# jackie840129/FedFR

Measured on AMD Instinct MI355X. Metric: images/sec (iresnet100+CosFace train step, bs=128/GPU, 112x112), higher is better.
Workload: dtype fp16; 1 GPU; iresnet100 + CosFace(s=30,m=0.4) + dense 1000-class cosine head, full train step (fwd+bwd+momentum-SGD), batch 128/GPU, 112x112 synthetic faces, random-init weights, fp16 activations/weights with fp32 accumulate + fp32 master weights, fp32 head; global_batch=128, parallelism=1 client per GPU (FedAvg), dp1, clients=1

## Files before the change

fedfr_amd/csrc/gemm_nt_glds.hip:

```cpp
#include "nt_epilogue.h"

#ifndef NT_GLDS_NS
#define NT_GLDS_NS 4
#endif
namespace {
template <int N_>
__device__ __forceinline__ void wait_vmcnt() {
  asm volatile("s_waitcnt vmcnt(%0)" ::"n"(N_) : "memory");
}

template <int BM, int BN, int WM, int WN, int NS, bool CONV>
__global__ __launch_bounds__(64 * WM * WN) void gemm_nt_glds_kernel(GemmNT p_) {
  GemmNT p = p_;
  if (p.par_on == 2) {
    const int cls = 3 - (int)blockIdx.z;
    p.par_h = cls >> 1; p.par_w = cls & 1;
    p.ksteps_total = (1 + p.par_h) * (1 + p.par_w) * p.cpt;
    p.ksteps_per_split = p.ksteps_total;
  }
  constexpr int NW = WM * WN, NT = 64 * NW;
  constexpr int TM = BM / WM / 16, TN = BN / WN / 16;
  constexpr int A_BYTES = BM * 128, B_BYTES = BN * 128, STAGE = A_BYTES + B_BYTES;
  constexpr int AP = (BM / 8) / NW, BP = (BN / 8) / NW, PER = AP + BP;
  constexpr int NRD = TM + TN, NM = TM * TN;
  static_assert((BM / 8) % NW == 0 && (BN / 8) % NW == 0 && NS >= 3 && NS <= 5 && AP >= 1 && BP >= 1, "tile geometry");
  typedef __attribute__((address_space(3))) void* lds_ptr_t;
  extern __shared__ __attribute__((aligned(1024))) unsigned char smem[];

  const int tid = threadIdx.x, lane = tid & 63;
  const int wave = __builtin_amdgcn_readfirstlane(tid >> 6);
  const int wm = wave / WN, wn = wave % WN;
  const int lid = xcd_remap(blockIdx.x, gridDim.x);
  const int bn = lid % p.nbn, bm = lid / p.nbn;
  const int split = blockIdx.y;
  const int m0 = bm * BM, n0 = bn * BN;
  const int kt0 = split * p.ksteps_per_split;
  const int kt1 = min(kt0 + p.ksteps_per_split, p.ksteps_total);

  const int prow = lane >> 3, pch = (lane & 7) ^ prow;
  constexpr unsigned OOB = 0xfffffff0u;
  int a_hb[AP], a_wb[AP];
  unsigned a_base[AP];
  bool a_ok[AP];
#pragma unroll
  for (int j = 0; j < AP; ++j) {
    const int m = m0 + (j * NW + wave) * 8 + prow;
    a_ok[j] = m < p.M;
    if (CONV) {
      const int mm = a_ok[j] ? m : 0;
      const int hw = p.Ho * p.Wo;
      const int img = mm / hw, rem = mm - img * hw;
      int ho = rem / p.Wo, wo = rem - ho * p.Wo;
      if (p.par_on) {
        ho = 2 * ho + p.par_h;
        wo = 2 * wo + p.par_w;
      }
      a_hb[j] = ho * p.stride - p.pad;
      a_wb[j] = wo * p.stride - p.pad;
      a_base[j] = ((unsigned)(img * p.H * p.W) * (unsigned)p.C + (unsigned)(pch * 8)) * 2u;
    } else {
      a_hb[j] = a_wb[j] = 0;
      a_base[j] = ((unsigned)(a_ok[j] ? m : 0) * (unsigned)p.lda + (unsigned)(pch * 8)) * 2u;
    }
  }
  unsigned b_base[BP];
  bool b_ok[BP];
#pragma unroll
  for (int j = 0; j < BP; ++j) {
    const int n = n0 + (j * NW + wave) * 8 + prow;
    b_ok[j] = n < p.N;
    b_base[j] = ((unsigned)(b_ok[j] ? n : 0) * (unsigned)p.K + (unsigned)(pch * 8)) * 2u;
  }
  int kti = kt0;
  int tap = kt0 / p.cpt, cc = kt0 - tap * p.cpt;
  int r = tap / p.S, s = tap - r * p.S;
  const int s0 = p.par_on ? 1 - p.par_w : 0, tstep = p.par_on ? 2 : 1;
  if (p.par_on) {
    const int nS = 1 + p.par_w;
    r = (1 - p.par_h) + 2 * (tap / nS);
    s = s0 + 2 * (tap % nS);
  }
  const __amdgpu_buffer_rsrc_t rsA = make_rsrc(p.A, p.a_bytes), rsB = make_rsrc(p.B, p.b_bytes);
  const int upm = p.up - 1, ups = p.up >> 1;
  const unsigned rowB = (unsigned)(p.W * p.C * 2), pixB = (unsigned)(p.C * 2);
  auto issue = [&](int slot) {
    unsigned char* sA = smem + slot * STAGE;
    unsigned char* sB = sA + A_BYTES;
    const bool live = kti < kt1;
    const unsigned kA = (unsigned)(CONV ? cc * 128 : kti * 128);
    const bool klive = live & (CONV | (kti * 64 + pch * 8 < p.K));
#pragma unroll
    for (int j = 0; j < AP; ++j) {
      bool ok = klive & a_ok[j];
      unsigned off = a_base[j] + kA;
      if (CONV) {
        int hp = a_hb[j] + r, wp = a_wb[j] + s;
        ok = ok & (((hp | wp) & upm) == 0);
        hp >>= ups;
        wp >>= ups;
        ok = ok & ((unsigned)hp < (unsigned)p.H) & ((unsigned)wp < (unsigned)p.W);
        off += __umul24((unsigned)hp, rowB) + __umul24((unsigned)wp, pixB);
      }
      __builtin_amdgcn_raw_ptr_buffer_load_lds(rsA, (lds_ptr_t)(sA + (j * NW + wave) * 1024), 16, (int)(ok ? off : OOB), 0, 0, 0);
    }
    const unsigned kB = (unsigned)(CONV ? ((r * p.S + s) * p.cpt + cc) * 128 : kti * 128);
#pragma unroll
    for (int j = 0; j < BP; ++j)
      __builtin_amdgcn_raw_ptr_buffer_load_lds(rsB, (lds_ptr_t)(sB + (j * NW + wave) * 1024), 16, (int)((klive & b_ok[j]) ? b_base[j] + kB : OOB), 0, 0, 0);
    ++kti;
    cc += 1;
    const bool wc = cc == p.cpt;
    cc = wc ? 0 : cc;
    s += wc ? tstep : 0;
    const bool ws = s >= p.S;
    s = ws ? s0 : s;
    r += ws ? tstep : 0;
  };

  const int l15 = lane & 15, lg = lane >> 4;
  int a_addr[TM], b_addr[TN];
#pragma unroll
  for (int mi = 0; mi < TM; ++mi) {
    const int row = wm * (BM / WM) + mi * 16 + l15;
    a_addr[mi] = row * 128 + ((lg ^ (row & 7)) << 4);
  }
#pragma unroll
  for (int ni = 0; ni < TN; ++ni) {
    const int row = wn * (BN / WN) + ni * 16 + l15;
    b_addr[ni] = A_BYTES + row * 128 + ((lg ^ (row & 7)) << 4);
  }
  f32x4_t acc[TN][TM];
#pragma unroll
  for (int a = 0; a < TN; ++a)
#pragma unroll
    for (int b = 0; b < TM; ++b) acc[a][b] = (f32x4_t){0.f, 0.f, 0.f, 0.f};
  bf16x8_t f0a[TM], f0b[TN], f1a[TM], f1b[TN];
  auto read_frags = [&](bf16x8_t (&fa)[TM], bf16x8_t (&fb)[TN], const unsigned char* st, int ks) {
#pragma unroll
    for (int ni = 0; ni < TN; ++ni) fb[ni] = *reinterpret_cast<const bf16x8_t*>(st + (b_addr[ni] ^ (ks * 64)));
#pragma unroll
    for (int mi = 0; mi < TM; ++mi) fa[mi] = *reinterpret_cast<const bf16x8_t*>(st + (a_addr[mi] ^ (ks * 64)));
  };
  auto mfma_all = [&](const bf16x8_t (&fa)[TM], const bf16x8_t (&fb)[TN]) {
#pragma unroll
    for (int ni = 0; ni < TN; ++ni)
#pragma unroll
      for (int mi = 0; mi < TM; ++mi) acc[ni][mi] = MFMA16(fb[ni], fa[mi], acc[ni][mi]);
  };

#pragma unroll
  for (int i = 0; i < NS - 1; ++i) issue(i);
  wait_vmcnt<(NS - 2) * PER>();
  __builtin_amdgcn_s_barrier();
  read_frags(f0a, f0b, smem, 0);
  int slot = 0;
  for (int kt = kt0; kt < kt1; ++kt) {
    const unsigned char* cur = smem + slot * STAGE;
    const int nslot = slot + 1 == NS ? 0 : slot + 1, fslot = slot == 0 ? NS - 1 : slot - 1;
    read_frags(f1a, f1b, cur, 1);
    mfma_all(f0a, f0b);
#pragma unroll
    for (int i = 0; i < NRD; ++i) {
      __builtin_amdgcn_sched_group_barrier(0x008, (NM / NRD) > 0 ? (NM / NRD) : 1, 0);
      __builtin_amdgcn_sched_group_barrier(0x100, 1, 0);
    }
    __builtin_amdgcn_sched_barrier(0);
    wait_vmcnt<(NS - 3) * PER>();
    __builtin_amdgcn_s_barrier();
    __builtin_amdgcn_sched_barrier(0);
    read_frags(f0a, f0b, smem + nslot * STAGE, 0);
    issue(fslot);
    mfma_all(f1a, f1b);
    constexpr int NE = NRD > PER ? NRD : PER, MP2 = (NM / NE) > 0 ? (NM / NE) : 1;
#pragma unroll
    for (int i = 0; i < NE; ++i) {
      __builtin_amdgcn_sched_group_barrier(0x008, MP2, 0);
      if (i < NRD) __builtin_amdgcn_sched_group_barrier(0x100, 1, 0);
      if (i < PER) __builtin_amdgcn_sched_group_barrier(0x020, 1, 0);
    }
    __builtin_amdgcn_sched_barrier(0);
    slot = nslot;
  }
  wait_vmcnt<0>();
  __syncthreads();
  nt_epilogue<BM, BN, WM, WN, NT>(p, acc, smem, bm, m0, n0, split, wm, wn, tid, lane);
}

template <int BM, int BN, int WM, int WN, int NS, bool CONV>
int launch_impl2(GemmNT p, int splits, int slot, hipStream_t st) {
  const int nbm = ceil_div(p.M, BM);
  p.nbn = ceil_div(p.N, BN);
  p.ksteps_per_split = ceil_div(p.ksteps_total, splits);
  FEDFR_REQUIRE(ceil_div(p.ksteps_total, p.ksteps_per_split) == splits, "gemm_nt_glds: splits=%d leaves an empty split (ksteps=%d)", splits,
                p.ksteps_total);
  constexpr size_t kRing = (size_t)NS * (BM + BN) * 128, kEpi = (size_t)BM * (BN * 2 + 16);
  constexpr size_t lds = kRing > kEpi ? kRing : kEpi;
  static PerDeviceOnce attr_once;
  attr_once.run([&] {
    hipFuncSetAttribute(reinterpret_cast<const void*>(&gemm_nt_glds_kernel<BM, BN, WM, WN, NS, CONV>), hipFuncAttributeMaxDynamicSharedMemorySize, (int)lds);
  });
  const dim3 grid(nbm * p.nbn, splits, p.par_on == 2 ? 4 : 1);
  ProfScope prof(slot, 2.0 * p.M * p.N * (p.par_on == 2 ? 64.0 * 9 * p.cpt : p.par_on ? 64.0 * p.ksteps_total : (double)p.K), st, gemm_nt_alg_bytes(p, splits));
  hipLaunchKernelGGL((gemm_nt_glds_kernel<BM, BN, WM, WN, NS, CONV>), grid, dim3(64 * WM * WN), lds, st, p);
  FEDFR_LAUNCH_CHECK("gemm_nt_glds");
  return FEDFR_OK;
}
template <int BM, int BN, int WM, int WN, int NS>
int launch_impl(const GemmNT& p, int splits, int slot, hipStream_t st) {
  if (p.mode == 1) {
    FEDFR_REQUIRE((long long)p.W * p.C * 2 < (1 << 24) && p.H < (1 << 15), "gemm_nt_glds: image row too large for the 24-bit address multiplies");
    return launch_impl2<BM, BN, WM, WN, NS, true>(p, splits, slot, st);
  }
  return launch_impl2<BM, BN, WM, WN, NS, false>(p, splits, slot, st);
}
}

int g_nt_glds = 4;

bool gemm_nt_glds_applies(const GemmNT& p, int BM, int splits) {
  const bool pays = (g_nt_glds & 8) || (!p.par_on && ceil_div(p.ksteps_total, splits) >= 16);
  return (g_nt_glds & 7) > 0 && p.N > 64 && (BM == 128 || BM == 64) && pays && !p.bpart && !p.esc && !p.eadd && !p.Cb2;
}

int launch_nt_glds(const GemmNT& p, int BM, int splits, int slot, hipStream_t st) {
  FEDFR_REQUIRE(gemm_nt_glds_applies(p, BM, splits), "gemm_nt_glds: unsupported problem");
  const int v = g_nt_glds & 7;
  const bool up = v >= 3 && BM == 64 && (!p.stats || ceil_div(p.M, 64) == 2 * ceil_div(p.M, 128));
  if (BM == 128 || up) return (v & 1) == 0 ? launch_impl<128, 128, 2, 4, NT_GLDS_NS>(p, splits, slot, st) : launch_impl<128, 128, 2, 2, 4>(p, splits, slot, st);
  return launch_impl<64, 128, 1, 4, 3>(p, splits, slot, st);
}
```

fedfr_amd/csrc/wgrad9.hip:

```cpp
#include "gemm_tn_dev.h"
#ifndef W9_READS_FIRST
#define W9_READS_FIRST 0
#endif
#ifndef W9_ABLATE
#define W9_ABLATE 0
#endif

int g_wgrad9 = 1;

namespace {
template <int N_>
__device__ __forceinline__ void w9_wait_vmcnt() {
  asm volatile("s_waitcnt vmcnt(%0)" ::"n"(N_) : "memory");
}
__device__ __forceinline__ int w9_swz(int row) { return (((row >> 1) & 1) << 1) | (((row >> 3) & 1) << 2); }

struct W9 {
  const bf16_t* dy;
  const bf16_t* x;
  float* out;
  int cout, cin, nci;
  int ntiles;
  int nstages, per_split;
  int W, lg;
  unsigned dy_bytes, x_bytes;
};

template <int W_, int R_, int LOG_PW>
__global__ __launch_bounds__(512) __attribute__((amdgpu_waves_per_eu(3, 3))) void wgrad9_kernel(W9 p) {
  constexpr int PW = 1 << LOG_PW, KP = R_ * PW, KS = KP / 32;
  constexpr int VG = PW / 16, WIN = 2 + 2 * VG, NG = 2 * KS + 2 * VG;
  constexpr int BANDS = W_ / R_;
  constexpr int P_PIECES = KP / 16;
  constexpr int Q_ROWS = (NG * 16 + 2 + 7) / 8 * 8, Q_PIECES = Q_ROWS / 8;
  constexpr int NP = P_PIECES + Q_PIECES, NPW = (NP + 7) / 8;
  constexpr int P_B = KP * 64, Q_B = Q_ROWS * 128, STAGE_B = P_B + Q_B;
  static_assert(KP % 32 == 0 && W_ % R_ == 0 && W_ <= PW && (R_ + 2) * PW + 2 <= Q_ROWS, "band geometry");
  static_assert(P_B % 1024 == 0 && (NG - 1) * 2048 < 65536, "ds_read immediate offsets");
  typedef __attribute__((address_space(3))) void* lds_ptr_t;
  typedef __attribute__((address_space(3))) unsigned char* lds_uc_t;
  extern __shared__ __attribute__((aligned(1024))) unsigned char smem[];

  const int tid = threadIdx.x, lane = tid & 63;
  const int wave = __builtin_amdgcn_readfirstlane(tid >> 6);
  const int cb = wave >> 1, ch = wave & 1;
  const int lid = xcd_remap((int)blockIdx.x, (int)gridDim.x);
  const int split = lid / p.ntiles, tile = lid - split * p.ntiles;
  const int tco = tile / p.nci, tci = tile - tco * p.nci;
  const int co0 = tco * 32, ci0 = tci * 64;
  const int s0 = split * p.per_split;
  const int nst = min(p.per_split, p.nstages - s0);

  const __amdgpu_buffer_rsrc_t rsP = make_rsrc(p.dy, p.dy_bytes), rsQ = make_rsrc(p.x, p.x_bytes);
  constexpr unsigned OOB = 0xfffffff0u;
  const int prow = lane >> 3;
  auto issue_stage = [&](int s, int buf) {
    const int per_img = BANDS << (2 * p.lg);
    const int img = s / per_img, rem = s - img * per_img;
    const int sub = rem / BANDS, band = rem - sub * BANDS;
    const int y0 = (sub >> p.lg) * W_ + band * R_, x0 = (sub & ((1 << p.lg) - 1)) * W_;
    const int Wi = p.W;
#pragma unroll
    for (int j = 0; j < NPW; ++j) {
      const int piece = min(j * 8 + wave, NP - 1);
      if (piece < P_PIECES) {
        const int r = piece * 16 + (lane >> 2);
        const int yl = r >> LOG_PW, xx = r & (PW - 1);
        const bool ok = s >= 0 && xx < W_;
        const unsigned off = ((unsigned)((img * Wi + y0 + yl) * Wi + x0 + xx) * (unsigned)p.cout + (unsigned)(co0 + (lane & 3) * 8)) * 2u;
        __builtin_amdgcn_raw_ptr_buffer_load_lds(rsP, (lds_ptr_t)(smem + buf * STAGE_B + piece * 1024), 16, (int)(ok ? off : OOB), 0, 0, 0);
      } else {
        const int qp = piece - P_PIECES;
        const int r = qp * 8 + prow;
        const int ql = r >> LOG_PW, xx = r & (PW - 1);
        const int lc = (lane & 7) ^ w9_swz(r);
        const int y = y0 + ql - 1, xc = x0 + xx - 1;
        const bool ok = s >= 0 && ql < R_ + 2 && xx < W_ + 2 && (unsigned)y < (unsigned)Wi && (unsigned)xc < (unsigned)Wi;
        const unsigned off = ((unsigned)((img * Wi + y) * Wi + xc) * (unsigned)p.cin + (unsigned)(ci0 + lc * 8)) * 2u;
        __builtin_amdgcn_raw_ptr_buffer_load_lds(rsQ, (lds_ptr_t)(smem + buf * STAGE_B + P_B + qp * 1024), 16, (int)(ok ? off : OOB), 0, 0, 0);
      }
    }
  };

  const int g = lane >> 4, q4 = (lane & 15) >> 2, pp = lane & 3;
  const unsigned lds0 = (unsigned)(size_t)(lds_uc_t)smem;
  auto frag_off = [&](int u, int colblk) {
    const int col = colblk + 4 * pp;
    return (unsigned)(u * 128 + (((col >> 3) ^ w9_swz(u)) << 4) + ((col >> 2) & 1) * 8);
  };
  unsigned offQ[3];
  const unsigned offP = lds0 + (unsigned)((4 * g + q4) * 64 + (ch * 16 + 4 * pp) * 2);
#pragma unroll
  for (int tx = 0; tx < 3; ++tx) offQ[tx] = lds0 + P_B + frag_off(tx + 4 * g + q4, cb * 16);

  f32x4_t acc[9];
#pragma unroll
  for (int t = 0; t < 9; ++t) acc[t] = (f32x4_t){0.f, 0.f, 0.f, 0.f};

  typedef __attribute__((ext_vector_type(2))) unsigned u32x2_t;
#define W9_READ(dst, addr, imm) asm volatile("ds_read_b64_tr_b16 %0, %1 offset:%2" : "=v"(dst) : "v"(addr), "n"(imm))
  u32x2_t Pf[2 * KS], Qg[3][NG];
  auto frag = [](const u32x2_t& lo, const u32x2_t& hi) {
    const u32x4_t v = {lo[0], lo[1], hi[0], hi[1]};
    return __builtin_bit_cast(bf16x8_t, v);
  };

  issue_stage(s0, 0);
  issue_stage(nst > 1 ? s0 + 1 : -1, 1);
  w9_wait_vmcnt<NPW>();
  __builtin_amdgcn_s_barrier();
  __builtin_amdgcn_sched_barrier(0);
#pragma unroll
  for (int j = 0; j < 2; ++j) W9_READ(Pf[j], offP, j * 1024);
#pragma unroll
  for (int tx = 0; tx < 3; ++tx)
#pragma unroll
    for (int j = 0; j < WIN; ++j) W9_READ(Qg[tx][j], offQ[tx], j * 2048);
  asm volatile("s_waitcnt lgkmcnt(0)" ::: "memory");
  __builtin_amdgcn_sched_barrier(0);

  for (int it = 0; it < nst; ++it) {
    const unsigned cur = (unsigned)((it & 1) * STAGE_B), nxt = (unsigned)(((it + 1) & 1) * STAGE_B);
    unsigned aQ[3], nQ[3];
    const unsigned aP = offP + cur, nP = offP + nxt;
#pragma unroll
    for (int tx = 0; tx < 3; ++tx) { aQ[tx] = offQ[tx] + cur; nQ[tx] = offQ[tx] + nxt; }
#pragma unroll
    for (int kb = 0; kb < KS; ++kb) {
      constexpr int NRL = 2 + 3 * WIN;
      const bool last = kb == KS - 1;
      if (last) {
        w9_wait_vmcnt<0>();
        if (!(W9_ABLATE & 8)) __builtin_amdgcn_s_barrier();
        __builtin_amdgcn_sched_barrier(0);
        if (!(W9_ABLATE & 1)) issue_stage(it + 2 < nst ? s0 + it + 2 : -1, it & 1);
        __builtin_amdgcn_sched_barrier(0);
      }
      auto issue_read = [&](int r) {
        if (W9_ABLATE & 2) return;
        if (!last) {
          if (r < 2) W9_READ(Pf[2 * kb + 2 + r], aP, (2 * kb + 2 + r) * 1024);
          else { const int tx = (r - 2) >> 1, j = 2 * kb + WIN + ((r - 2) & 1); W9_READ(Qg[tx][j], aQ[tx], j * 2048); }
        } else {
          if (r < 2) W9_READ(Pf[r], nP, r * 1024);
          else { const int tx = (r - 2) / WIN, j = (r - 2) % WIN; W9_READ(Qg[tx][j], nQ[tx], j * 2048); }
        }
      };
      const int nr = last ? NRL : 8;
      const int r0 = W9_READS_FIRST ? nr : (last ? NRL - 9 : 0);
#pragma unroll
      for (int r = 0; r < NRL; ++r)
        if (r < r0) issue_read(r);
      __builtin_amdgcn_sched_barrier(0);
#pragma unroll
      for (int ty = 0; ty < 3; ++ty)
#pragma unroll
        for (int tx = 0; tx < 3; ++tx) {
          const int m = ty * 3 + tx;
          if (!(W9_ABLATE & 4)) acc[m] = MFMA16(frag(Qg[tx][2 * kb + ty * VG], Qg[tx][2 * kb + ty * VG + 1]), frag(Pf[2 * kb], Pf[2 * kb + 1]), acc[m]);
          if (r0 + m < nr) issue_read(r0 + m);
          __builtin_amdgcn_sched_barrier(0);
        }
      asm volatile("s_waitcnt lgkmcnt(0)" ::: "memory");
      __builtin_amdgcn_sched_barrier(0);
    }
  }
#undef W9_READ
  w9_wait_vmcnt<0>();

  float* slab = p.out + (size_t)split * p.cout * 9 * p.cin;
  const int NJ = 9 * p.cin;
  const int co = co0 + ch * 16 + (lane & 15);
  const int ci = ci0 + cb * 16 + (lane >> 4) * 4;
#pragma unroll
  for (int t = 0; t < 9; ++t)
    if (!(W9_ABLATE & 16) || acc[t][0] == 12345.f)
      *reinterpret_cast<float4*>(slab + (size_t)co * NJ + t * p.cin + ci) = make_float4(acc[t][0], acc[t][1], acc[t][2], acc[t][3]);
}

template <int W_, int R_, int LOG_PW>
constexpr size_t w9_lds() {
  constexpr int PW = 1 << LOG_PW, KP = R_ * PW, KS = KP / 32, VG = PW / 16, NG = 2 * KS + 2 * VG;
  return 2 * (size_t)(KP * 64 + (NG * 16 + 2 + 7) / 8 * 8 * 128);
}
}

extern int g_tn_use_tr;
static int w9_lg(int W) {
  for (int lg = 0; lg < 4; ++lg)
    if (W == (14 << lg)) return lg;
  return -1;
}
bool wgrad9_shape_ok(int Kp, int NI, int NJ, int C, int W, int stride) {
  return stride == 1 && w9_lg(W) >= 0 && C > 0 && C % 64 == 0 && NI % 32 == 0 && NJ == 9 * C && Kp % (W * W) == 0;
}
bool wgrad9_applies_shape(int Kp, int NI, int NJ, int C, int W, int stride) {
  return g_wgrad9 && g_tn_use_tr && wgrad9_shape_ok(Kp, NI, NJ, C, W, stride);
}
bool wgrad9_applies(const GemmTN& p) {
  return p.mode == 1 && p.use_tr && p.S == 3 && p.pad == 1 && p.H == p.W && p.Ho == p.H && p.Wo == p.W && p.ldp == p.NI &&
         wgrad9_applies_shape(p.Kp, p.NI, p.NJ, p.C, p.W, p.stride);
}
static int w9_stages(int Kp, int W) {
  const int images = Kp / (W * W);
  return images << (2 * w9_lg(W));
}
static const int g_wgrad9_wgs = 256;
int wgrad9_pick_splits(int Kp, int NI, int NJ, int W) {
  const int stages = w9_stages(Kp, W);
  const int tiles = (NI / 32) * (NJ / 9 / 64);
  int splits = g_wgrad9_wgs / tiles;
  if (splits < 1) splits = 1;
  if (splits > stages / 2) splits = stages / 2 > 0 ? stages / 2 : 1;
  const int per = ceil_div(stages, splits);
  return ceil_div(stages, per);
}

int launch_wgrad9(const GemmTN& g, int splits, hipStream_t st) {
  FEDFR_REQUIRE(wgrad9_applies(g), "wgrad9: unsupported problem");
  W9 p{};
  p.dy = g.P; p.x = g.Q; p.out = g.out; p.cout = g.NI; p.cin = g.C; p.nci = g.C / 64;
  p.ntiles = (g.NI / 32) * p.nci;
  p.W = g.W; p.lg = w9_lg(g.W);
  p.nstages = w9_stages(g.Kp, g.W);
  p.per_split = ceil_div(p.nstages, splits);
  FEDFR_REQUIRE(splits >= 1 && ceil_div(p.nstages, p.per_split) == splits, "wgrad9: splits=%d leaves an empty split", splits);
  p.dy_bytes = g.p_bytes; p.x_bytes = g.q_bytes;
  const dim3 grid(p.ntiles * splits);
  ProfScope prof(16, 2.0 * g.NI * g.NJ * (double)g.Kp, st, gemm_tn_alg_bytes(g, 1));
  constexpr size_t lds14 = w9_lds<14, 14, 4>();
  static PerDeviceOnce attr_once;
  attr_once.run([&] {
    hipFuncSetAttribute(reinterpret_cast<const void*>(&wgrad9_kernel<14, 14, 4>), hipFuncAttributeMaxDynamicSharedMemorySize, (int)lds14);
  });
  hipLaunchKernelGGL((wgrad9_kernel<14, 14, 4>), grid, dim3(512), lds14, st, p);
  FEDFR_LAUNCH_CHECK("wgrad9");
  return FEDFR_OK;
}
```

Measured before the change: 8438 images/sec.

## Add image-resident LDS path for 7x7 3x3 convs and reswizzle wgrad9 LDS

Adds a resident variant of the implicit-GEMM conv kernel for 7x7 stride-1 3x3 convolutions. Each block loads its whole padded image tile (up to four images) into LDS once per channel chunk and serves all nine taps from it by shifting fragment addresses, double-buffering image chunks while a separate ring streams the weights. The goal is to remove the ninefold re-fetch of activation tiles per tap, at the cost of more LDS per block and a complex wait-count schedule. Separately, it changes the XOR swizzle of the wgrad9 LDS layouts for both operands, aiming to cut LDS bank conflicts on the transposed reads.

```diff
diff --git a/fedfr_amd/csrc/gemm_nt_glds.hip b/fedfr_amd/csrc/gemm_nt_glds.hip
--- a/fedfr_amd/csrc/gemm_nt_glds.hip
+++ b/fedfr_amd/csrc/gemm_nt_glds.hip
@@ -1,7 +1,11 @@
 #include "nt_epilogue.h"
+#include "nt_resident_plan.h"
 
 #ifndef NT_GLDS_NS
 #define NT_GLDS_NS 4
+#endif
+#ifndef NT_GLDS_RESIDENT
+#define NT_GLDS_RESIDENT 1
 #endif
 namespace {
 template <int N_>
@@ -9,8 +13,151 @@
   asm volatile("s_waitcnt vmcnt(%0)" ::"n"(N_) : "memory");
 }
 
-template <int BM, int BN, int WM, int WN, int NS, bool CONV>
+template <int BM, int BN, int WM, int WN, int NS>
+__device__ __forceinline__ void nt_resident_body(const GemmNT& p, unsigned char* smem) {
+  constexpr int NW = WM * WN, NT = 64 * NW;
+  constexpr int TM = BM / WM / 16, TN = BN / WN / 16;
+  constexpr int IMG_B = ntr::kImgBytes, RING0 = 2 * IMG_B, B_BYTES = BN * 128;
+  constexpr int BP = (BN / 8) / NW, AIP = ntr::img_per_wave(NW);
+  constexpr int NRD = TM + TN, NM = TM * TN;
+  static_assert(BM == 128 && (BN / 8) % NW == 0 && BP >= 1 && NS >= 3 && NS <= 5, "tile geometry");
+  static_assert(ntr::img_first(ntr::kTaps, AIP, NS) == AIP, "a chunk's image pieces are all issued within its taps");
+  static_assert(ntr::lds_bytes(NS, BN) <= 160 * 1024 && BM * (BN * 2 + 16) <= ntr::lds_bytes(NS, BN), "two image buffers + B ring, and the epilogue's staging tile, within LDS");
+  typedef __attribute__((address_space(3))) void* lds_ptr_t;
+
+  const int tid = threadIdx.x, lane = tid & 63;
+  const int wave = __builtin_amdgcn_readfirstlane(tid >> 6);
+  const int wm = wave / WN, wn = wave % WN;
+  const int lid = xcd_remap(blockIdx.x, gridDim.x);
+  const int bn = lid % p.nbn, bm = lid / p.nbn;
+  const int split = blockIdx.y;
+  const int m0 = bm * BM, n0 = bn * BN;
+  const int c0 = split * (p.ksteps_per_split / ntr::kTaps);
+  const int c1 = min(c0 + p.ksteps_per_split / ntr::kTaps, p.cpt);
+
+  const int prow = lane >> 3, pch = ntr::piece_chunk(lane);
+  constexpr unsigned OOB = 0xfffffff0u;
+  const int img0 = m0 / ntr::kPix;
+  const int nimgs = min(p.M / ntr::kPix, (m0 + BM - 1) / ntr::kPix + 1) - img0;
+  unsigned a_src[AIP];
+#pragma unroll
+  for (int j = 0; j < AIP; ++j) {
+    const int pix = ntr::piece_pixel(ntr::wave_piece(j, wave, NW), prow, nimgs);
+    a_src[j] = pix < 0 ? OOB : ((unsigned)(img0 * ntr::kPix + pix) * (unsigned)p.C + (unsigned)(pch * 8)) * 2u;
+  }
+  unsigned b_base[BP];
+  bool b_ok[BP];
+#pragma unroll
+  for (int j = 0; j < BP; ++j) {
+    const int n = n0 + (j * NW + wave) * 8 + prow;
+    b_ok[j] = n < p.N;
+    b_base[j] = ((unsigned)(b_ok[j] ? n : 0) * (unsigned)p.K + (unsigned)(pch * 8)) * 2u;
+  }
+  const __amdgpu_buffer_rsrc_t rsA = make_rsrc(p.A, p.a_bytes), rsB = make_rsrc(p.B, p.b_bytes);
+  auto issue_img = [&](int j, int buf, int cc) {
+    const bool ok = (cc < c1) & (a_src[j] != OOB);
+    __builtin_amdgcn_raw_ptr_buffer_load_lds(rsA, (lds_ptr_t)(smem + buf * IMG_B + ntr::piece_lds(ntr::wave_piece(j, wave, NW))), 16,
+                                             (int)(ok ? a_src[j] + (unsigned)cc * 128u : OOB), 0, 0, 0);
+  };
+  auto issue_b = [&](int slot, int cc, int tap) {
+    const bool live = cc < c1;
+    const unsigned kB = (unsigned)((tap * p.cpt + cc) * 128);
+#pragma unroll
+    for (int j = 0; j < BP; ++j)
+      __builtin_amdgcn_raw_ptr_buffer_load_lds(rsB, (lds_ptr_t)(smem + RING0 + slot * B_BYTES + (j * NW + wave) * 1024), 16,
+                                               (int)((live & b_ok[j]) ? b_base[j] + kB : OOB), 0, 0, 0);
+  };
+
+  const int l15 = lane & 15, lg = lane >> 4;
+  int a_res[3][TM], b_addr[TN];
+#pragma unroll
+  for (int mi = 0; mi < TM; ++mi) {
+    const int u = ntr::pos_of(m0 + wm * (BM / WM) + mi * 16 + l15, img0);
+#pragma unroll
+    for (int s = 0; s < 3; ++s) a_res[s][mi] = ntr::frag_addr(u, s, lg);
+  }
+#pragma unroll
+  for (int ni = 0; ni < TN; ++ni) {
+    const int row = wn * (BN / WN) + ni * 16 + l15;
+    b_addr[ni] = RING0 + row * 128 + ((lg ^ (row & 7)) << 4);
+  }
+  f32x4_t acc[TN][TM];
+#pragma unroll
+  for (int a = 0; a < TN; ++a)
+#pragma unroll
+    for (int b = 0; b < TM; ++b) acc[a][b] = (f32x4_t){0.f, 0.f, 0.f, 0.f};
+  bf16x8_t f0a[TM], f0b[TN], f1a[TM], f1b[TN];
+  auto read_frags = [&](bf16x8_t (&fa)[TM], bf16x8_t (&fb)[TN], const unsigned char* sb, const unsigned char* sa, int tap, int ks) {
+#pragma unroll
+    for (int ni = 0; ni < TN; ++ni) fb[ni] = *reinterpret_cast<const bf16x8_t*>(sb + (b_addr[ni] ^ (ks * 64)));
+#pragma unroll
+    for (int mi = 0; mi < TM; ++mi) fa[mi] = *reinterpret_cast<const bf16x8_t*>(sa + (a_res[tap % 3][mi] ^ (ks * 64)) + (tap / 3) * ntr::kRowStep);
+  };
+  auto mfma_all = [&](const bf16x8_t (&fa)[TM], const bf16x8_t (&fb)[TN]) {
+#pragma unroll
+    for (int ni = 0; ni < TN; ++ni)
+#pragma unroll
+      for (int mi = 0; mi < TM; ++mi) acc[ni][mi] = MFMA16(fb[ni], fa[mi], acc[ni][mi]);
+  };
+
+#pragma unroll
+  for (int j = 0; j < AIP; ++j) issue_img(j, 0, c0);
+#pragma unroll
+  for (int i = 0; i < NS - 1; ++i) issue_b(i, c0 + i / ntr::kTaps, i % ntr::kTaps);
+  wait_vmcnt<(NS - 2) * BP>();
+  __builtin_amdgcn_s_barrier();
+  read_frags(f0a, f0b, smem, smem, 0, 0);
+  int slot = 0;
+  for (int c = c0; c < c1; ++c) {
+    const int obuf = ((c - c0) & 1) ^ 1;
+    const unsigned char* curA = smem + (obuf ^ 1) * IMG_B;
+    const unsigned char* othA = smem + obuf * IMG_B;
+    auto step = [&](auto T_) __attribute__((always_inline)) {
+      constexpr int t = decltype(T_)::value;
+      const int nslot = slot + 1 == NS ? 0 : slot + 1, fslot = slot == 0 ? NS - 1 : slot - 1;
+      read_frags(f1a, f1b, smem + slot * B_BYTES, curA, t, 1);
+      mfma_all(f0a, f0b);
+#pragma unroll
+      for (int i = 0; i < NRD; ++i) {
+        __builtin_amdgcn_sched_group_barrier(0x008, (NM / NRD) > 0 ? (NM / NRD) : 1, 0);
+        __builtin_amdgcn_sched_group_barrier(0x100, 1, 0);
+      }
+      __builtin_amdgcn_sched_barrier(0);
+      wait_vmcnt<ntr::wait_n(t, BP, AIP, NS)>();
+      __builtin_amdgcn_s_barrier();
+      __builtin_amdgcn_sched_barrier(0);
+      read_frags(f0a, f0b, smem + nslot * B_BYTES, t == ntr::kTaps - 1 ? othA : curA, (t + 1) % ntr::kTaps, 0);
+      constexpr int NCNT = ntr::img_cnt(t, AIP, NS), NFIRST = ntr::img_first(t, AIP, NS);
+#pragma unroll
+      for (int j = NFIRST; j < NFIRST + NCNT; ++j) issue_img(j, obuf, c + 1);
+      issue_b(fslot, c + (t + NS - 1) / ntr::kTaps, (t + NS - 1) % ntr::kTaps);
+      mfma_all(f1a, f1b);
+      constexpr int PER = BP + NCNT, NE = NRD > PER ? NRD : PER, MP2 = (NM / NE) > 0 ? (NM / NE) : 1;
+#pragma unroll
+      for (int i = 0; i < NE; ++i) {
+        __builtin_amdgcn_sched_group_barrier(0x008, MP2, 0);
+        if (i < NRD) __builtin_amdgcn_sched_group_barrier(0x100, 1, 0);
+        if (i < PER) __builtin_amdgcn_sched_group_barrier(0x020, 1, 0);
+      }
+      __builtin_amdgcn_sched_barrier(0);
+      slot = nslot;
+    };
+    step(std::integral_constant<int, 0>{}); step(std::integral_constant<int, 1>{}); step(std::integral_constant<int, 2>{});
+    step(std::integral_constant<int, 3>{}); step(std::integral_constant<int, 4>{}); step(std::integral_constant<int, 5>{});
+    step(std::integral_constant<int, 6>{}); step(std::integral_constant<int, 7>{}); step(std::integral_constant<int, 8>{});
+  }
+  wait_vmcnt<0>();
+  __syncthreads();
+  nt_epilogue<BM, BN, WM, WN, NT>(p, acc, smem, bm, m0, n0, split, wm, wn, tid, lane);
+}
+
+template <int BM, int BN, int WM, int WN, int NS, bool CONV, bool RES = false>
 __global__ __launch_bounds__(64 * WM * WN) void gemm_nt_glds_kernel(GemmNT p_) {
+  if constexpr (RES) {
+    extern __shared__ __attribute__((aligned(1024))) unsigned char smem_res[];
+    nt_resident_body<BM, BN, WM, WN, NS>(p_, smem_res);
+    return;
+  }
   GemmNT p = p_;
   if (p.par_on == 2) {
     const int cls = 3 - (int)blockIdx.z;
@@ -186,22 +333,22 @@
   nt_epilogue<BM, BN, WM, WN, NT>(p, acc, smem, bm, m0, n0, split, wm, wn, tid, lane);
 }
 
-template <int BM, int BN, int WM, int WN, int NS, bool CONV>
+template <int BM, int BN, int WM, int WN, int NS, bool CONV, bool RES = false>
 int launch_impl2(GemmNT p, int splits, int slot, hipStream_t st) {
   const int nbm = ceil_div(p.M, BM);
   p.nbn = ceil_div(p.N, BN);
   p.ksteps_per_split = ceil_div(p.ksteps_total, splits);
   FEDFR_REQUIRE(ceil_div(p.ksteps_total, p.ksteps_per_split) == splits, "gemm_nt_glds: splits=%d leaves an empty split (ksteps=%d)", splits,
                 p.ksteps_total);
-  constexpr size_t kRing = (size_t)NS * (BM + BN) * 128, kEpi = (size_t)BM * (BN * 2 + 16);
+  constexpr size_t kRing = RES ? (size_t)ntr::lds_bytes(NS, BN) : (size_t)NS * (BM + BN) * 128, kEpi = (size_t)BM * (BN * 2 + 16);
   constexpr size_t lds = kRing > kEpi ? kRing : kEpi;
   static PerDeviceOnce attr_once;
   attr_once.run([&] {
-    hipFuncSetAttribute(reinterpret_cast<const void*>(&gemm_nt_glds_kernel<BM, BN, WM, WN, NS, CONV>), hipFuncAttributeMaxDynamicSharedMemorySize, (int)lds);
+    hipFuncSetAttribute(reinterpret_cast<const void*>(&gemm_nt_glds_kernel<BM, BN, WM, WN, NS, CONV, RES>), hipFuncAttributeMaxDynamicSharedMemorySize, (int)lds);
   });
   const dim3 grid(nbm * p.nbn, splits, p.par_on == 2 ? 4 : 1);
   ProfScope prof(slot, 2.0 * p.M * p.N * (p.par_on == 2 ? 64.0 * 9 * p.cpt : p.par_on ? 64.0 * p.ksteps_total : (double)p.K), st, gemm_nt_alg_bytes(p, splits));
-  hipLaunchKernelGGL((gemm_nt_glds_kernel<BM, BN, WM, WN, NS, CONV>), grid, dim3(64 * WM * WN), lds, st, p);
+  hipLaunchKernelGGL((gemm_nt_glds_kernel<BM, BN, WM, WN, NS, CONV, RES>), grid, dim3(64 * WM * WN), lds, st, p);
   FEDFR_LAUNCH_CHECK("gemm_nt_glds");
   return FEDFR_OK;
 }
@@ -209,6 +356,13 @@
 int launch_impl(const GemmNT& p, int splits, int slot, hipStream_t st) {
   if (p.mode == 1) {
     FEDFR_REQUIRE((long long)p.W * p.C * 2 < (1 << 24) && p.H < (1 << 15), "gemm_nt_glds: image row too large for the 24-bit address multiplies");
+    if constexpr (NT_GLDS_RESIDENT && BM == 128) {
+      const int per = ceil_div(p.ksteps_total, splits);
+      if (p.S == 3 && p.K == 9 * p.C && p.stride == 1 && p.pad == 1 && !p.par_on && p.up == 1 && p.H == ntr::kSide && p.W == ntr::kSide &&
+          p.Ho == ntr::kSide && p.Wo == ntr::kSide && p.C % 64 == 0 && p.cpt == p.C / 64 && p.ksteps_total == ntr::kTaps * p.cpt &&
+          p.M % ntr::kPix == 0 && per % ntr::kTaps == 0)
+        return launch_impl2<BM, BN, WM, WN, NS, true, true>(p, splits, slot, st);
+    }
     return launch_impl2<BM, BN, WM, WN, NS, true>(p, splits, slot, st);
   }
   return launch_impl2<BM, BN, WM, WN, NS, false>(p, splits, slot, st);
diff --git a/fedfr_amd/csrc/nt_resident_plan.h b/fedfr_amd/csrc/nt_resident_plan.h
--- /dev/null
+++ b/fedfr_amd/csrc/nt_resident_plan.h
@@ -0,0 +1,48 @@
+#pragma once
+#if defined(__HIPCC__)
+#define NTR_FN __host__ __device__ inline
+#else
+#define NTR_FN inline
+#endif
+
+namespace ntr {
+constexpr int kSide = 7, kPix = kSide * kSide, kTaps = 9;
+constexpr int kPitch = 8, kImgPos = 64, kMaxImgs = 4;
+constexpr int kPieces = kMaxImgs * 8 + 2;
+constexpr int kPos = kPieces * kPitch;
+constexpr int kImgBytes = kPos * 128;
+constexpr int kRowStep = kPitch * 128;
+
+NTR_FN constexpr int pos_of(int m, int img0) {
+  return (m / kPix - img0) * kImgPos + ((m % kPix) / kSide + 1) * kPitch + (m % kPix) % kSide + 1;
+}
+NTR_FN constexpr int tap_shift(int r, int s) { return (r - 1) * kPitch + (s - 1); }
+
+NTR_FN constexpr int piece_pixel(int q, int prow, int nimgs) {
+  return (prow == 0 || (q & 7) == 0 || (q >> 3) >= nimgs) ? -1 : (q >> 3) * kPix + ((q & 7) - 1) * kSide + prow - 1;
+}
+NTR_FN constexpr int piece_chunk(int lane) { return (lane & 7) ^ (lane >> 3); }
+NTR_FN constexpr int piece_lds(int q) { return q * 1024; }
+NTR_FN constexpr int wave_piece(int j, int wave, int nw) {
+  return j * nw + wave < kPieces ? j * nw + wave : kPieces - 1;
+}
+
+NTR_FN constexpr int frag_addr(int u, int s, int lg) {
+  return (u + s - 1 - kPitch) * 128 + ((lg ^ ((u + s - 1) & 7)) << 4);
+}
+
+NTR_FN constexpr int img_per_wave(int nw) { return (kPieces + nw - 1) / nw; }
+NTR_FN constexpr int img_taps(int ns) { return kTaps + 2 - ns; }
+NTR_FN constexpr int img_cnt(int tap, int aip, int ns) { return tap < img_taps(ns) ? (aip + img_taps(ns) - 1 - tap) / img_taps(ns) : 0; }
+NTR_FN constexpr int img_first(int tap, int aip, int ns) {
+  int n = 0;
+  for (int t = 0; t < tap; ++t) n += img_cnt(t, aip, ns);
+  return n;
+}
+NTR_FN constexpr int wait_n(int tap, int bp, int aip, int ns) {
+  int n = 0;
+  for (int d = 1; d <= ns - 3; ++d) n += bp + img_cnt((tap + kTaps - d) % kTaps, aip, ns);
+  return n;
+}
+NTR_FN constexpr int lds_bytes(int ns, int bn) { return 2 * kImgBytes + ns * bn * 128; }
+}
diff --git a/fedfr_amd/csrc/wgrad9.hip b/fedfr_amd/csrc/wgrad9.hip
--- a/fedfr_amd/csrc/wgrad9.hip
+++ b/fedfr_amd/csrc/wgrad9.hip
@@ -13,7 +13,11 @@
 __device__ __forceinline__ void w9_wait_vmcnt() {
   asm volatile("s_waitcnt vmcnt(%0)" ::"n"(N_) : "memory");
 }
-__device__ __forceinline__ int w9_swz(int row) { return (((row >> 1) & 1) << 1) | (((row >> 3) & 1) << 2); }
+#ifndef W9_SWZ_OLD
+#define W9_SWZ_OLD 0
+#endif
+__device__ __forceinline__ int w9_swz(int row) { return W9_SWZ_OLD ? ((((row >> 1) & 1) << 1) | (((row >> 3) & 1) << 2)) : (((row >> 1) & 3) << 1); }
+__device__ __forceinline__ int w9_swzP(int row) { return W9_SWZ_OLD ? 0 : (((row >> 2) & 1) << 1); }
 
 struct W9 {
   const bf16_t* dy;
@@ -67,7 +71,7 @@
         const int r = piece * 16 + (lane >> 2);
         const int yl = r >> LOG_PW, xx = r & (PW - 1);
         const bool ok = s >= 0 && xx < W_;
-        const unsigned off = ((unsigned)((img * Wi + y0 + yl) * Wi + x0 + xx) * (unsigned)p.cout + (unsigned)(co0 + (lane & 3) * 8)) * 2u;
+        const unsigned off = ((unsigned)((img * Wi + y0 + yl) * Wi + x0 + xx) * (unsigned)p.cout + (unsigned)(co0 + ((lane & 3) ^ w9_swzP(r)) * 8)) * 2u;
         __builtin_amdgcn_raw_ptr_buffer_load_lds(rsP, (lds_ptr_t)(smem + buf * STAGE_B + piece * 1024), 16, (int)(ok ? off : OOB), 0, 0, 0);
       } else {
         const int qp = piece - P_PIECES;
@@ -89,7 +93,7 @@
     return (unsigned)(u * 128 + (((col >> 3) ^ w9_swz(u)) << 4) + ((col >> 2) & 1) * 8);
   };
   unsigned offQ[3];
-  const unsigned offP = lds0 + (unsigned)((4 * g + q4) * 64 + (ch * 16 + 4 * pp) * 2);
+  const unsigned offP = lds0 + (unsigned)((4 * g + q4) * 64 + (((ch * 2 + (pp >> 1)) ^ w9_swzP(4 * g + q4)) << 4) + (pp & 1) * 8);
 #pragma unroll
   for (int tx = 0; tx < 3; ++tx) offQ[tx] = lds0 + P_B + frag_off(tx + 4 * g + q4, cb * 16);
 
```

Result: no change. 8469 images/sec (median of 6 runs) (+0.4%).
